# iiscleap/ICL-speech-text-LLM

Hardware: AMD Instinct MI355X
Metric: ICL utterances/sec (whole node), SALMONN+Llama2-7B 5-shot VOXCELEB (higher is better)
Workload: dtype bf16

## Files before the change

### icl-speech-text-llm_amd/csrc/gemm256.hip

```cpp
#include "gemm_common.h"
#include <cstdlib>

using namespace iclg;

#ifndef ICL_EPI_NT
#define ICL_EPI_NT 3
#endif

namespace {

constexpr int T256_REGION = 128 * 128;
constexpr int T256_BUF = 4 * T256_REGION;
constexpr int T256_SMEM = 256 * (256 * 2 + 16);

__device__ __forceinline__ void st16(unsigned short* dst, u32x4 v) {
  if (ICL_EPI_NT & 4) __builtin_nontemporal_store(v, (u32x4*)dst);
  else *(u32x4*)dst = v;
}

__device__ __forceinline__ void rope_rows(const GemmParams& p, const RopeFuse& rf, const char* smem, int pitch, int m0,
                                          int n0, int tid) {
  const int sect = n0 >= rf.v_off ? 2 : (n0 >= rf.k_off ? 1 : 0);
  const int head0 = (n0 - (sect == 2 ? rf.v_off : sect == 1 ? rf.k_off : 0)) >> 7;
  unsigned short* C = (unsigned short*)p.C;
  constexpr int U = 4;
  if (sect == 2) {
    for (int base = tid; base < 256 * 32; base += U * 512) {
      int64_t crow[U];
      if (rf.vc) {
#pragma unroll
        for (int u = 0; u < U; ++u) {
          const int m = min(m0 + ((base + u * 512) >> 5), p.M - 1);
          crow[u] = (int64_t)rf.seq_ids[m] * rf.H * rf.max_len + rf.pos[m];
        }
      }
#pragma unroll
      for (int u = 0; u < U; ++u) {
        const int c = base + u * 512, row = c >> 5, cc = c & 31, m = m0 + row;
        if (m >= p.M) continue;
        const u32x4 v = *(const u32x4*)(smem + row * pitch + cc * 16);
        if (rf.kv_rows_to_c) st16(C + (int64_t)m * p.ldc + n0 + cc * 8, v);
        if (rf.vc) st16(rf.vc + (crow[u] + (int64_t)(head0 + (cc >> 4)) * rf.max_len) * 128 + (cc & 15) * 8, v);
      }
    }
    return;
  }
  const bool to_cache = sect == 1 && rf.kc;
  for (int base = tid; base < 256 * 16; base += U * 512) {
    int ps[U], sq[U];
    u32x4 lo[U], hi[U];
    f32x4 c0[U], c1[U], s0[U], s1[U];
#pragma unroll
    for (int u = 0; u < U; ++u) {
      const int m = min(m0 + ((base + u * 512) >> 4), p.M - 1);
      ps[u] = rf.pos[m];
      sq[u] = to_cache ? rf.seq_ids[m] : 0;
    }
#pragma unroll
    for (int u = 0; u < U; ++u) {
      const int it = base + u * 512, row = it >> 4, hh = (it >> 3) & 1, j = it & 7;
      const char* src = smem + row * pitch + hh * 256 + j * 16;
      lo[u] = *(const u32x4*)src;
      hi[u] = *(const u32x4*)(src + 128);
      const float* cp = rf.cosT + (int64_t)ps[u] * 64 + j * 8;
      const float* sp = rf.sinT + (int64_t)ps[u] * 64 + j * 8;
      c0[u] = *(const f32x4*)cp;
      c1[u] = *(const f32x4*)(cp + 4);
      s0[u] = *(const f32x4*)sp;
      s1[u] = *(const f32x4*)(sp + 4);
    }
#pragma unroll
    for (int u = 0; u < U; ++u) {
      const int it = base + u * 512, row = it >> 4, hh = (it >> 3) & 1, j = it & 7, m = m0 + row;
      if (m >= p.M) continue;
      u32x4 olo, ohi;
      rope_rot8(lo[u], hi[u], c0[u], c1[u], s0[u], s1[u], olo, ohi);
      if (sect == 0 || rf.kv_rows_to_c) {
        unsigned short* dst = C + (int64_t)m * p.ldc + n0 + hh * 128 + j * 8;
        st16(dst, olo);
        st16(dst + 64, ohi);
      }
      if (to_cache) {
        unsigned short* cd = rf.kc + (((int64_t)sq[u] * rf.H + head0 + hh) * rf.max_len + ps[u]) * 128 + j * 8;
        st16(cd, olo);
        st16(cd + 64, ohi);
      }
    }
  }
}

constexpr int T256_OUT_F32 = 16;
template <bool ROPE, int EPI>
__global__ __launch_bounds__(512, 2) void gemm256_bf16_kernel(GemmParams p_in, RopeFuse rf) {
  GemmParams p = p_in;
  p.epi = (p_in.epi & ICL_EPI_BIAS) | (EPI & (ICL_EPI_GELU | ICL_EPI_RESIDUAL | ICL_EPI_SWIGLU));
  p.out_dtype = (EPI & T256_OUT_F32) ? ICL_F32 : ICL_BF16;
  extern __shared__ __attribute__((aligned(16))) char smem[];
  const int tid = threadIdx.x, lane = tid & 63;
  const int wave = __builtin_amdgcn_readfirstlane(tid >> 6);
  const int wr = wave >> 2, wc = wave & 3;
  int tm, tn;
  block_to_tile(p, blockIdx.x, tm, tn);
  const int m0 = tm * 256, n0 = tn * 256;
  int z = blockIdx.z;
  int nk = p.K >> 6, kt0 = 0;
  const bool slab_out = p.split_k > 1;
  if (p.split_k > 1) {
    kt0 = (int)(((int64_t)z * nk) / p.split_k);
    nk = (int)(((int64_t)(z + 1) * nk) / p.split_k) - kt0;
    p.C = p.ws + (int64_t)z * p.M * p.N;
    p.ldc = p.N;
    p.sC = 0;
    p.epi = 0;
    z = 0;
  }
  const __bf16* A = p.A + (int64_t)z * p.sA + (int64_t)kt0 * 64;
  const __bf16* Wk = p.W + (int64_t)kt0 * 64;

  const __bf16* gsrc[2][2][2];
#pragma unroll
  for (int h = 0; h < 2; ++h)
#pragma unroll
    for (int r = 0; r < 2; ++r) {
      const int row = (r * 8 + wave) * 8 + (lane >> 3);
      const int chunk = (lane & 7) ^ ((row >> 1) & 7);
      gsrc[0][h][r] = A + (int64_t)min(m0 + h * 128 + row, p.M - 1) * p.lda + chunk * 8;
      gsrc[1][h][r] = Wk + (int64_t)min(n0 + h * 128 + row, p.N - 1) * p.ldw + chunk * 8;
    }
  auto stage = [&](int bo, int which, int h, int kt) {
    const int64_t koff = (int64_t)min(kt, nk - 1) * 64;
    char* base = smem + bo + (which * 2 + h) * T256_REGION + wave * 1024;
    __builtin_amdgcn_global_load_lds((gptr_t)(gsrc[which][h][0] + koff), (lptr_t)(base), 16, 0, 0);
    __builtin_amdgcn_global_load_lds((gptr_t)(gsrc[which][h][1] + koff), (lptr_t)(base + 8 * 1024), 16, 0, 0);
  };

  const int fr = lane & 15, fq = lane >> 4;
  const int a_base = (wr * 64 + fr) * 128, b_base = (wc * 32 + fr) * 128;
  const int sw0 = ((0 + fq) ^ (fr >> 1)) * 16, sw1 = ((4 + fq) ^ (fr >> 1)) * 16;

  f32x4 acc[2][2][4][2];
#pragma unroll
  for (int a = 0; a < 2; ++a)
#pragma unroll
    for (int b = 0; b < 2; ++b)
#pragma unroll
      for (int i = 0; i < 4; ++i)
#pragma unroll
        for (int j = 0; j < 2; ++j) acc[a][b][i][j] = f32x4{0.f, 0.f, 0.f, 0.f};
  bf16x8 af[4][2], b0f[2][2], b1f[2][2];
  const bool vecp = vec_path_ok(p);
  const bool interior = vecp && (m0 + 256 <= p.M) && (n0 + 256 <= p.N);
  const bool fold_bias = vecp && (p.epi & ICL_EPI_BIAS);
  constexpr bool fold_res = false;

  auto read_a = [&](int bo, int h) {
    const char* r = smem + bo + h * T256_REGION + a_base;
#pragma unroll
    for (int i = 0; i < 4; ++i) {
      af[i][0] = *(const bf16x8*)(r + i * 2048 + sw0);
      af[i][1] = *(const bf16x8*)(r + i * 2048 + sw1);
    }
  };
  auto read_b = [&](int bo, int h, bf16x8 (&bf)[2][2]) {
    const char* r = smem + bo + (2 + h) * T256_REGION + b_base;
#pragma unroll
    for (int j = 0; j < 2; ++j) {
      bf[j][0] = *(const bf16x8*)(r + j * 2048 + sw0);
      bf[j][1] = *(const bf16x8*)(r + j * 2048 + sw1);
    }
  };
  auto mma = [&](f32x4 (&c)[4][2], bf16x8 (&bf)[2][2]) {
    __builtin_amdgcn_s_setprio(1);
#pragma unroll
    for (int kk = 0; kk < 2; ++kk)
#pragma unroll
      for (int i = 0; i < 4; ++i)
#pragma unroll
        for (int j = 0; j < 2; ++j)
          c[i][j] = __builtin_amdgcn_mfma_f32_16x16x32_bf16(bf[j][kk], af[i][kk], c[i][j], 0, 0, 0);
    __builtin_amdgcn_s_setprio(0);
    __builtin_amdgcn_sched_barrier(0);
    __builtin_amdgcn_s_barrier();
    __builtin_amdgcn_sched_barrier(0);
  };
  auto phase_sync = [&](auto n_tag) {
    constexpr int N = decltype(n_tag)::value;
    if constexpr (N == 8) asm volatile("s_waitcnt vmcnt(8)" ::: "memory");
    else if constexpr (N == 6) asm volatile("s_waitcnt vmcnt(6)" ::: "memory");
    else if constexpr (N == 4) asm volatile("s_waitcnt vmcnt(4)" ::: "memory");
    else if constexpr (N == 2) asm volatile("s_waitcnt vmcnt(2)" ::: "memory");
    else asm volatile("s_waitcnt vmcnt(0)" ::: "memory");
    __builtin_amdgcn_sched_barrier(0);
    __builtin_amdgcn_s_barrier();
    __builtin_amdgcn_sched_barrier(0);
  };
  auto tile = [&](int bo, int t, auto mode) {
    constexpr int MODE = decltype(mode)::value;
    const int bx = bo ^ T256_BUF;
    read_a(bo, 0);
    read_b(bo, 0, b0f);
    if constexpr (MODE != 2) stage(bx, 1, 1, t + 1);
    phase_sync(std::integral_constant<int, MODE == 2 ? 2 : 8>{});
    mma(acc[0][0], b0f);
    read_b(bo, 1, b1f);
    if constexpr (MODE != 2) stage(bx, 0, 1, t + 1);
    phase_sync(std::integral_constant<int, MODE == 2 ? 0 : 8>{});
    mma(acc[0][1], b1f);
    read_a(bo, 1);
    if constexpr (MODE == 0) stage(bo, 0, 0, t + 2);
    phase_sync(std::integral_constant<int, MODE == 0 ? 8 : (MODE == 1 ? 6 : 0)>{});
    mma(acc[1][1], b1f);
    if constexpr (MODE == 0) stage(bo, 1, 0, t + 2);
    phase_sync(std::integral_constant<int, MODE == 0 ? 8 : (MODE == 1 ? 4 : 0)>{});
    mma(acc[1][0], b0f);
  };
  using M0_ = std::integral_constant<int, 0>;
  using M1_ = std::integral_constant<int, 1>;
  using M2_ = std::integral_constant<int, 2>;

  f32x4 bias_f[2][2];
  if (fold_res) {
#pragma unroll
    for (int qa = 0; qa < 2; ++qa)
#pragma unroll
      for (int qb = 0; qb < 2; ++qb)
#pragma unroll
        for (int i = 0; i < 4; ++i)
#pragma unroll
          for (int j = 0; j < 2; ++j) {
            const int m = m0 + qa * 128 + wr * 64 + i * 16 + fr, n = n0 + qb * 128 + wc * 32 + j * 16 + fq * 4;
            if (interior || (m < p.M && n < p.N))
              acc[qa][qb][i][j] = *(const f32x4*)((const float*)p.R + (int64_t)z * p.sR + (int64_t)m * p.ldr + n);
          }
  }
  if (fold_bias) {
#pragma unroll
    for (int qb = 0; qb < 2; ++qb)
#pragma unroll
      for (int j = 0; j < 2; ++j) {
        const int n = n0 + qb * 128 + wc * 32 + j * 16 + fq * 4;
        bias_f[qb][j] = (interior || n < p.N) ? *(const f32x4*)(p.bias + n) : f32x4{0.f, 0.f, 0.f, 0.f};
      }
  }
  __builtin_amdgcn_sched_barrier(0);
  stage(0, 0, 0, 0);
  stage(0, 1, 0, 0);
  stage(0, 1, 1, 0);
  stage(0, 0, 1, 0);
  stage(T256_BUF, 0, 0, 1);
  stage(T256_BUF, 1, 0, 1);
  __builtin_amdgcn_sched_barrier(0);
  if (fold_bias) {
#pragma unroll
    for (int qa = 0; qa < 2; ++qa)
#pragma unroll
      for (int qb = 0; qb < 2; ++qb)
#pragma unroll
        for (int i = 0; i < 4; ++i)
#pragma unroll
          for (int j = 0; j < 2; ++j) acc[qa][qb][i][j] = acc[qa][qb][i][j] + bias_f[qb][j];
  }
  phase_sync(std::integral_constant<int, 8>{});
  if (wr == 1) __builtin_amdgcn_s_barrier();
  const int n_steady = nk - 2;
  int t = 0;
  for (; t + 1 < n_steady; t += 2) {
    tile(0, t, M0_{});
    tile(T256_BUF, t + 1, M0_{});
  }
  if (t < n_steady) {
    tile(0, t, M0_{});
    ++t;
  }
  const int bo = (t & 1) ? T256_BUF : 0;
  tile(bo, t, M1_{});
  tile(bo ^ T256_BUF, t + 1, M2_{});
  if (wr == 0) __builtin_amdgcn_s_barrier();

  const int es_out = p.out_dtype == ICL_BF16 ? 2 : 4;
  const bool rows16 = (((uintptr_t)p.C | (uintptr_t)(p.ldc * es_out) | (uintptr_t)(p.sC * es_out)) & 15) == 0;
  const bool has_res = p.epi & ICL_EPI_RESIDUAL;
  const bool res_rows = has_res && p.res_dtype == ICL_F32 && p.out_dtype == ICL_F32 && !(p.epi & ICL_EPI_SWIGLU) &&
                        (((uintptr_t)p.R | (uintptr_t)(p.ldr * 4) | (uintptr_t)(p.sR * 4)) & 15) == 0;
  if (ROPE || (interior && rows16 && (!has_res || res_rows))) {
    const bool swiglu = p.epi & ICL_EPI_SWIGLU;
    const bool obf = p.out_dtype == ICL_BF16;
    const int out_cols = swiglu ? 128 : 256;
    const int es = obf ? 2 : 4;
    const int pitch = out_cols * es + 16;
    const int chunks_per_row = out_cols * es / 16;
    const int64_t c_col0 = swiglu ? (n0 >> 1) : n0;
    const bool one_round = ROPE || obf;
    f32x4 rrA[16], rrB[16];
    auto load_res_rows = [&](int qa_, f32x4 (&rr)[16]) {
      const char* rbase = (const char*)p.R + ((int64_t)z * p.sR + (int64_t)(m0 + qa_ * 128) * p.ldr + n0) * 4;
#pragma unroll
      for (int it = 0; it < 16; ++it) {
        const int c = tid + it * 512, row = c >> 6, cc = c & 63;
        rr[it] = ICL_EPI_NT & 1 ? __builtin_nontemporal_load((const f32x4*)(rbase + (int64_t)row * p.ldr * 4 + cc * 16))
                                : *(const f32x4*)(rbase + (int64_t)row * p.ldr * 4 + cc * 16);
      }
    };
    if (has_res) load_res_rows(0, rrA);
#pragma unroll
    for (int qa = 0; qa < 2; ++qa) {
      if (qa == 0 || !one_round) __syncthreads();
      const int row_off = one_round ? qa * 128 : 0;
#pragma unroll
      for (int qb = 0; qb < 2; ++qb)
#pragma unroll
        for (int i = 0; i < 4; ++i) {
          const int row = row_off + wr * 64 + i * 16 + fr;
          if (swiglu) {
            f32x4 v;
#pragma unroll
            for (int r = 0; r < 4; ++r) v[r] = silu_f(acc[qa][qb][i][0][r]) * acc[qa][qb][i][1][r];
            const int col = qb * 64 + wc * 16 + fq * 4;
            char* dst = smem + row * pitch + col * es;
            if (obf) *(u32x2*)dst = u32x2{pack_bf16x2(v[0], v[1]), pack_bf16x2(v[2], v[3])};
            else *(f32x4*)dst = v;
          } else {
#pragma unroll
            for (int j = 0; j < 2; ++j) {
              f32x4 v = acc[qa][qb][i][j];
              if (p.epi & ICL_EPI_GELU) {
            v = gelu_erf4(v);
              }
              const int col = qb * 128 + wc * 32 + j * 16 + fq * 4;
              char* dst = smem + row * pitch + col * es;
              if (obf) *(u32x2*)dst = u32x2{pack_bf16x2(v[0], v[1]), pack_bf16x2(v[2], v[3])};
              else *(f32x4*)dst = v;
            }
          }
        }
      if (one_round && qa == 0) continue;
      __syncthreads();
      if constexpr (ROPE) {
        rope_rows(p, rf, smem, pitch, m0, n0, tid);
        continue;
      }
      char* cbase = (char*)p.C + ((int64_t)z * p.sC + (int64_t)(m0 + (one_round ? 0 : qa * 128)) * p.ldc + c_col0) * es;
      const int n_chunks = (one_round ? 256 : 128) * chunks_per_row;
      if (has_res) {
        if (qa == 0) load_res_rows(1, rrB);
        f32x4 (&rr)[16] = qa == 0 ? rrA : rrB;
#pragma unroll
        for (int it = 0; it < 16; ++it) {
          const int c = tid + it * 512, row = c >> 6, cc = c & 63;
          const f32x4 v = *(const f32x4*)(smem + row * pitch + cc * 16) + rr[it];
          if (ICL_EPI_NT & 1) __builtin_nontemporal_store(v, (f32x4*)(cbase + (int64_t)row * p.ldc * 4 + cc * 16));
          else *(f32x4*)(cbase + (int64_t)row * p.ldc * 4 + cc * 16) = v;
        }
      } else {
        const int n_iter = n_chunks >> 9;
        u32x4 v[16];
#pragma unroll
        for (int it = 0; it < 16; ++it)
          if (it < n_iter) {
            const int c = tid + it * 512, row = c / chunks_per_row, cc = c - row * chunks_per_row;
            v[it] = *(const u32x4*)(smem + row * pitch + cc * 16);
          }
#pragma unroll
        for (int it = 0; it < 16; ++it)
          if (it < n_iter) {
            const int c = tid + it * 512, row = c / chunks_per_row, cc = c - row * chunks_per_row;
            if ((ICL_EPI_NT & 2) && !slab_out) __builtin_nontemporal_store(v[it], (u32x4*)(cbase + (int64_t)row * p.ldc * es + cc * 16));
            else *(u32x4*)(cbase + (int64_t)row * p.ldc * es + cc * 16) = v[it];
          }
      }
    }
    return;
  } else if (interior) {
    const bool late_res = (p.epi & ICL_EPI_RESIDUAL) && !fold_res;
#pragma unroll
    for (int qa = 0; qa < 2; ++qa) {
      const int mb = m0 + qa * 128 + wr * 64 + fr;
      if (p.epi & ICL_EPI_SWIGLU) {
#pragma unroll
        for (int i = 0; i < 4; ++i)
#pragma unroll
          for (int qb = 0; qb < 2; ++qb) {
            f32x4 v;
#pragma unroll
            for (int r = 0; r < 4; ++r) v[r] = silu_f(acc[qa][qb][i][0][r]) * acc[qa][qb][i][1][r];
            store_out4(p, (int64_t)z * p.sC + (int64_t)(mb + i * 16) * p.ldc + ((n0 + qb * 128 + wc * 32) >> 1) + fq * 4, v);
          }
        continue;
      }
      f32x4 rv[2][4][2];
      if (late_res) {
#pragma unroll
        for (int qb = 0; qb < 2; ++qb)
#pragma unroll
          for (int i = 0; i < 4; ++i)
#pragma unroll
            for (int j = 0; j < 2; ++j)
              rv[qb][i][j] = load_res4(p, (int64_t)z * p.sR + (int64_t)(mb + i * 16) * p.ldr + n0 + qb * 128 + wc * 32 + j * 16 + fq * 4);
      }
#pragma unroll
      for (int qb = 0; qb < 2; ++qb)
#pragma unroll
        for (int i = 0; i < 4; ++i)
#pragma unroll
          for (int j = 0; j < 2; ++j) {
            f32x4 v = acc[qa][qb][i][j];
            if (p.epi & ICL_EPI_GELU) {
            v = gelu_erf4(v);
            }
            if (late_res) v = v + rv[qb][i][j];
            store_out4(p, (int64_t)z * p.sC + (int64_t)(mb + i * 16) * p.ldc + n0 + qb * 128 + wc * 32 + j * 16 + fq * 4, v);
          }
    }
    return;
  }

  GemmParams q = p;
  if (fold_bias) q.epi &= ~ICL_EPI_BIAS;
  if (fold_res) q.epi &= ~ICL_EPI_RESIDUAL;
#pragma unroll
  for (int qa = 0; qa < 2; ++qa)
#pragma unroll
    for (int i = 0; i < 4; ++i) {
      const int m = m0 + qa * 128 + wr * 64 + i * 16 + fr;
#pragma unroll
      for (int qb = 0; qb < 2; ++qb) {
        const int nt = n0 + qb * 128 + wc * 32;
        if (p.epi & ICL_EPI_SWIGLU) {
          epi_store_swiglu(q, z, m, nt, fq * 4, acc[qa][qb][i][0], acc[qa][qb][i][1]);
        } else {
          epi_store4(q, z, m, nt + fq * 4, acc[qa][qb][i][0]);
          epi_store4(q, z, m, nt + 16 + fq * 4, acc[qa][qb][i][1]);
        }
      }
    }
}

template <bool ROPE, int EPI>
int launch256(const GemmParams& p, const dim3& grid, hipStream_t stream, const RopeFuse& rf) {
  auto kern = gemm256_bf16_kernel<ROPE, EPI>;
  static bool attr_set = false;
  if (!attr_set) {
    const hipError_t e = hipFuncSetAttribute((const void*)kern, hipFuncAttributeMaxDynamicSharedMemorySize, T256_SMEM);
    if (e != hipSuccess) {
      icl_set_error("icl_gemm_bf16: hipFuncSetAttribute(%d) failed: %s", T256_SMEM, hipGetErrorString(e));
      return ICL_ELAUNCH;
    }
    attr_set = true;
  }
  hipLaunchKernelGGL(kern, grid, dim3(512), T256_SMEM, stream, p, rf);
  ICL_CHECK_LAUNCH("icl_gemm_bf16(256)");
  return ICL_OK;
}

}

int iclg::launch_tile256(GemmParams& p, int batch, hipStream_t stream, const RopeFuse* rope) {
  p.tiles_m = (p.M + 255) / 256;
  p.tiles_n = (p.N + 255) / 256;
  {
    static const int env_gm = [] { const char* e = getenv("ICL_GEMM_GROUP_M"); return e ? atoi(e) : 0; }();
    static const int env_xs = [] { const char* e = getenv("ICL_GEMM_XCD_SYNC"); return e ? atoi(e) : 1; }();
    const int64_t panel = (int64_t)256 * p.K * 2;
    p.group_m = env_gm > 0 ? env_gm : (int)std::min<int64_t>(6, std::max<int64_t>(1, 8400000 / panel));
    p.xcd_sync = env_xs;
  }
  const dim3 grid(p.tiles_m * p.tiles_n, 1, p.split_k > 1 ? p.split_k : batch);
  if (rope) return launch256<true, 0>(p, grid, stream, *rope);
  const RopeFuse none{};
  constexpr int G = ICL_EPI_GELU, R = ICL_EPI_RESIDUAL, S = ICL_EPI_SWIGLU, F = T256_OUT_F32;
  if (p.split_k > 1) return launch256<false, F>(p, grid, stream, none);
  switch ((p.epi & (G | R | S)) | (p.out_dtype == ICL_F32 ? F : 0)) {
    case 0:         return launch256<false, 0>(p, grid, stream, none);
    case G:         return launch256<false, G>(p, grid, stream, none);
    case R:         return launch256<false, R>(p, grid, stream, none);
    case G | R:     return launch256<false, G | R>(p, grid, stream, none);
    case S:         return launch256<false, S>(p, grid, stream, none);
    case F:         return launch256<false, F>(p, grid, stream, none);
    case F | G:     return launch256<false, F | G>(p, grid, stream, none);
    case F | R:     return launch256<false, F | R>(p, grid, stream, none);
    case F | G | R: return launch256<false, F | G | R>(p, grid, stream, none);
    case F | S:     return launch256<false, F | S>(p, grid, stream, none);
  }
  icl_set_error("icl_gemm_bf16(256): unsupported epilogue combination 0x%x", p.epi);
  return ICL_EINVAL;
}
```

Measured before the change: 143.2.

## Make 256-tile GEMM persistent and overlap next tile prologue with epilogue stores

Turns the 256x256 GEMM kernel into a persistent kernel: the grid is capped at the CU count and each workgroup loops over tiles with stride gridDim.x. During the row-store epilogue of one tile, it resets the accumulators, loads the bias and issues the first global-to-LDS loads for the next tile. A new pipeline mode accounts for the extra outstanding stores in vmcnt. This hides the prologue latency and launch tail, but adds complexity and a fixed CU-count grid, which can unbalance the last wave of tiles.

```diff
diff --git a/icl-speech-text-llm_amd/csrc/gemm256.hip b/icl-speech-text-llm_amd/csrc/gemm256.hip
--- a/icl-speech-text-llm_amd/csrc/gemm256.hip
+++ b/icl-speech-text-llm_amd/csrc/gemm256.hip
@@ -95,13 +95,12 @@
   GemmParams p = p_in;
   p.epi = (p_in.epi & ICL_EPI_BIAS) | (EPI & (ICL_EPI_GELU | ICL_EPI_RESIDUAL | ICL_EPI_SWIGLU));
   p.out_dtype = (EPI & T256_OUT_F32) ? ICL_F32 : ICL_BF16;
+  constexpr int S_AFTER = ROPE ? 0 : ((EPI & T256_OUT_F32 ? 128 : 256) * ((EPI & ICL_EPI_SWIGLU ? 128 : 256) * (EPI & T256_OUT_F32 ? 4 : 2) / 16)) >> 9;
   extern __shared__ __attribute__((aligned(16))) char smem[];
-  const int tid = threadIdx.x, lane = tid & 63;
-  const int wave = __builtin_amdgcn_readfirstlane(tid >> 6);
+  const int wave = __builtin_amdgcn_readfirstlane(threadIdx.x >> 6);
   const int wr = wave >> 2, wc = wave & 3;
-  int tm, tn;
-  block_to_tile(p, blockIdx.x, tm, tn);
-  const int m0 = tm * 256, n0 = tn * 256;
+  const int nwg = p.tiles_m * p.tiles_n;
+  int bid = blockIdx.x;
   int z = blockIdx.z;
   int nk = p.K >> 6, kt0 = 0;
   const bool slab_out = p.split_k > 1;
@@ -117,16 +116,42 @@
   const __bf16* A = p.A + (int64_t)z * p.sA + (int64_t)kt0 * 64;
   const __bf16* Wk = p.W + (int64_t)kt0 * 64;
 
+  const bool vecp = vec_path_ok(p);
+  const bool fold_bias = vecp && (p.epi & ICL_EPI_BIAS);
+  constexpr bool fold_res = false;
+
+  int m0, n0;
+  bool interior;
   const __bf16* gsrc[2][2][2];
-#pragma unroll
-  for (int h = 0; h < 2; ++h)
-#pragma unroll
-    for (int r = 0; r < 2; ++r) {
-      const int row = (r * 8 + wave) * 8 + (lane >> 3);
-      const int chunk = (lane & 7) ^ ((row >> 1) & 7);
-      gsrc[0][h][r] = A + (int64_t)min(m0 + h * 128 + row, p.M - 1) * p.lda + chunk * 8;
-      gsrc[1][h][r] = Wk + (int64_t)min(n0 + h * 128 + row, p.N - 1) * p.ldw + chunk * 8;
-    }
+  f32x4 bias_f[2][2];
+  auto tile_begin = [&](int b) {
+    int tid = threadIdx.x;
+    asm volatile("" : "+v"(tid));
+    const int lane = tid & 63, fq = lane >> 4;
+    int tm, tn;
+    block_to_tile(p, b, tm, tn);
+    m0 = __builtin_amdgcn_readfirstlane(tm * 256);
+    n0 = __builtin_amdgcn_readfirstlane(tn * 256);
+    interior = vecp && (m0 + 256 <= p.M) && (n0 + 256 <= p.N);
+#pragma unroll
+    for (int h = 0; h < 2; ++h)
+#pragma unroll
+      for (int r = 0; r < 2; ++r) {
+        const int row = (r * 8 + wave) * 8 + (lane >> 3);
+        const int chunk = (lane & 7) ^ ((row >> 1) & 7);
+        gsrc[0][h][r] = A + (int64_t)min(m0 + h * 128 + row, p.M - 1) * p.lda + chunk * 8;
+        gsrc[1][h][r] = Wk + (int64_t)min(n0 + h * 128 + row, p.N - 1) * p.ldw + chunk * 8;
+      }
+    if (fold_bias) {
+#pragma unroll
+      for (int qb = 0; qb < 2; ++qb)
+#pragma unroll
+        for (int j = 0; j < 2; ++j) {
+          const int n = n0 + qb * 128 + wc * 32 + j * 16 + fq * 4;
+          bias_f[qb][j] = (interior || n < p.N) ? *(const f32x4*)(p.bias + n) : f32x4{0.f, 0.f, 0.f, 0.f};
+        }
+    }
+  };
   auto stage = [&](int bo, int which, int h, int kt) {
     const int64_t koff = (int64_t)min(kt, nk - 1) * 64;
     char* base = smem + bo + (which * 2 + h) * T256_REGION + wave * 1024;
@@ -134,24 +159,26 @@
     __builtin_amdgcn_global_load_lds((gptr_t)(gsrc[which][h][1] + koff), (lptr_t)(base + 8 * 1024), 16, 0, 0);
   };
 
+  const int lane = threadIdx.x & 63;
   const int fr = lane & 15, fq = lane >> 4;
   const int a_base = (wr * 64 + fr) * 128, b_base = (wc * 32 + fr) * 128;
   const int sw0 = ((0 + fq) ^ (fr >> 1)) * 16, sw1 = ((4 + fq) ^ (fr >> 1)) * 16;
 
   f32x4 acc[2][2][4][2];
-#pragma unroll
-  for (int a = 0; a < 2; ++a)
-#pragma unroll
-    for (int b = 0; b < 2; ++b)
-#pragma unroll
-      for (int i = 0; i < 4; ++i)
-#pragma unroll
-        for (int j = 0; j < 2; ++j) acc[a][b][i][j] = f32x4{0.f, 0.f, 0.f, 0.f};
   bf16x8 af[4][2], b0f[2][2], b1f[2][2];
-  const bool vecp = vec_path_ok(p);
-  const bool interior = vecp && (m0 + 256 <= p.M) && (n0 + 256 <= p.N);
-  const bool fold_bias = vecp && (p.epi & ICL_EPI_BIAS);
-  constexpr bool fold_res = false;
+  auto acc_init = [&] {
+#pragma unroll
+    for (int qa = 0; qa < 2; ++qa)
+#pragma unroll
+      for (int qb = 0; qb < 2; ++qb)
+#pragma unroll
+        for (int i = 0; i < 4; ++i)
+#pragma unroll
+          for (int j = 0; j < 2; ++j) {
+            acc[qa][qb][i][j] = f32x4{0.f, 0.f, 0.f, 0.f};
+            if (fold_bias) acc[qa][qb][i][j] = acc[qa][qb][i][j] + bias_f[qb][j];
+          }
+  };
 
   auto read_a = [&](int bo, int h) {
     const char* r = smem + bo + h * T256_REGION + a_base;
@@ -185,11 +212,8 @@
   };
   auto phase_sync = [&](auto n_tag) {
     constexpr int N = decltype(n_tag)::value;
-    if constexpr (N == 8) asm volatile("s_waitcnt vmcnt(8)" ::: "memory");
-    else if constexpr (N == 6) asm volatile("s_waitcnt vmcnt(6)" ::: "memory");
-    else if constexpr (N == 4) asm volatile("s_waitcnt vmcnt(4)" ::: "memory");
-    else if constexpr (N == 2) asm volatile("s_waitcnt vmcnt(2)" ::: "memory");
-    else asm volatile("s_waitcnt vmcnt(0)" ::: "memory");
+    static_assert(N >= 0 && N <= 63, "vmcnt is a 6-bit field on gfx950");
+    asm volatile("s_waitcnt vmcnt(%0)" ::"n"(N) : "memory");
     __builtin_amdgcn_sched_barrier(0);
     __builtin_amdgcn_s_barrier();
     __builtin_amdgcn_sched_barrier(0);
@@ -199,89 +223,46 @@
     const int bx = bo ^ T256_BUF;
     read_a(bo, 0);
     read_b(bo, 0, b0f);
+    constexpr int W8 = MODE == 3 ? 8 + S_AFTER : 8;
     if constexpr (MODE != 2) stage(bx, 1, 1, t + 1);
-    phase_sync(std::integral_constant<int, MODE == 2 ? 2 : 8>{});
+    phase_sync(std::integral_constant<int, MODE == 2 ? 2 : W8>{});
     mma(acc[0][0], b0f);
     read_b(bo, 1, b1f);
     if constexpr (MODE != 2) stage(bx, 0, 1, t + 1);
-    phase_sync(std::integral_constant<int, MODE == 2 ? 0 : 8>{});
+    phase_sync(std::integral_constant<int, MODE == 2 ? 0 : W8>{});
     mma(acc[0][1], b1f);
     read_a(bo, 1);
-    if constexpr (MODE == 0) stage(bo, 0, 0, t + 2);
-    phase_sync(std::integral_constant<int, MODE == 0 ? 8 : (MODE == 1 ? 6 : 0)>{});
+    if constexpr (MODE == 0 || MODE == 3) stage(bo, 0, 0, t + 2);
+    phase_sync(std::integral_constant<int, MODE == 0 || MODE == 3 ? W8 : (MODE == 1 ? 6 : 0)>{});
     mma(acc[1][1], b1f);
-    if constexpr (MODE == 0) stage(bo, 1, 0, t + 2);
-    phase_sync(std::integral_constant<int, MODE == 0 ? 8 : (MODE == 1 ? 4 : 0)>{});
+    if constexpr (MODE == 0 || MODE == 3) stage(bo, 1, 0, t + 2);
+    phase_sync(std::integral_constant<int, MODE == 0 || MODE == 3 ? W8 : (MODE == 1 ? 4 : 0)>{});
     mma(acc[1][0], b0f);
   };
   using M0_ = std::integral_constant<int, 0>;
   using M1_ = std::integral_constant<int, 1>;
   using M2_ = std::integral_constant<int, 2>;
-
-  f32x4 bias_f[2][2];
-  if (fold_res) {
-#pragma unroll
-    for (int qa = 0; qa < 2; ++qa)
-#pragma unroll
-      for (int qb = 0; qb < 2; ++qb)
-#pragma unroll
-        for (int i = 0; i < 4; ++i)
-#pragma unroll
-          for (int j = 0; j < 2; ++j) {
-            const int m = m0 + qa * 128 + wr * 64 + i * 16 + fr, n = n0 + qb * 128 + wc * 32 + j * 16 + fq * 4;
-            if (interior || (m < p.M && n < p.N))
-              acc[qa][qb][i][j] = *(const f32x4*)((const float*)p.R + (int64_t)z * p.sR + (int64_t)m * p.ldr + n);
-          }
-  }
-  if (fold_bias) {
-#pragma unroll
-    for (int qb = 0; qb < 2; ++qb)
-#pragma unroll
-      for (int j = 0; j < 2; ++j) {
-        const int n = n0 + qb * 128 + wc * 32 + j * 16 + fq * 4;
-        bias_f[qb][j] = (interior || n < p.N) ? *(const f32x4*)(p.bias + n) : f32x4{0.f, 0.f, 0.f, 0.f};
-      }
-  }
-  __builtin_amdgcn_sched_barrier(0);
-  stage(0, 0, 0, 0);
-  stage(0, 1, 0, 0);
-  stage(0, 1, 1, 0);
-  stage(0, 0, 1, 0);
-  stage(T256_BUF, 0, 0, 1);
-  stage(T256_BUF, 1, 0, 1);
-  __builtin_amdgcn_sched_barrier(0);
-  if (fold_bias) {
-#pragma unroll
-    for (int qa = 0; qa < 2; ++qa)
-#pragma unroll
-      for (int qb = 0; qb < 2; ++qb)
-#pragma unroll
-        for (int i = 0; i < 4; ++i)
-#pragma unroll
-          for (int j = 0; j < 2; ++j) acc[qa][qb][i][j] = acc[qa][qb][i][j] + bias_f[qb][j];
-  }
-  phase_sync(std::integral_constant<int, 8>{});
-  if (wr == 1) __builtin_amdgcn_s_barrier();
-  const int n_steady = nk - 2;
-  int t = 0;
-  for (; t + 1 < n_steady; t += 2) {
-    tile(0, t, M0_{});
-    tile(T256_BUF, t + 1, M0_{});
-  }
-  if (t < n_steady) {
-    tile(0, t, M0_{});
-    ++t;
-  }
-  const int bo = (t & 1) ? T256_BUF : 0;
-  tile(bo, t, M1_{});
-  tile(bo ^ T256_BUF, t + 1, M2_{});
-  if (wr == 0) __builtin_amdgcn_s_barrier();
+  using M3_ = std::integral_constant<int, 3>;
+
+  auto prologue = [&] {
+    __builtin_amdgcn_sched_barrier(0);
+    stage(0, 0, 0, 0);
+    stage(0, 1, 0, 0);
+    stage(0, 1, 1, 0);
+    stage(0, 0, 1, 0);
+    stage(T256_BUF, 0, 0, 1);
+    stage(T256_BUF, 1, 0, 1);
+    __builtin_amdgcn_sched_barrier(0);
+  };
 
   const int es_out = p.out_dtype == ICL_BF16 ? 2 : 4;
   const bool rows16 = (((uintptr_t)p.C | (uintptr_t)(p.ldc * es_out) | (uintptr_t)(p.sC * es_out)) & 15) == 0;
   const bool has_res = p.epi & ICL_EPI_RESIDUAL;
   const bool res_rows = has_res && p.res_dtype == ICL_F32 && p.out_dtype == ICL_F32 && !(p.epi & ICL_EPI_SWIGLU) &&
                         (((uintptr_t)p.R | (uintptr_t)(p.ldr * 4) | (uintptr_t)(p.sR * 4)) & 15) == 0;
+  auto epilogue = [&](const bool more, const int nbid) -> bool {
+  int tid = threadIdx.x;
+  asm volatile("" : "+v"(tid));
   if (ROPE || (interior && rows16 && (!has_res || res_rows))) {
     const bool swiglu = p.epi & ICL_EPI_SWIGLU;
     const bool obf = p.out_dtype == ICL_BF16;
@@ -302,6 +283,14 @@
       }
     };
     if (has_res) load_res_rows(0, rrA);
+    const bool prefetch = !ROPE && more && nk >= 4;
+    auto next_prologue = [&] {
+      acc_init();
+      asm volatile("s_waitcnt lgkmcnt(0)" ::: "memory");
+      __builtin_amdgcn_sched_barrier(0);
+      __builtin_amdgcn_s_barrier();
+      prologue();
+    };
 #pragma unroll
     for (int qa = 0; qa < 2; ++qa) {
       if (qa == 0 || !one_round) __syncthreads();
@@ -334,22 +323,30 @@
           }
         }
       if (one_round && qa == 0) continue;
+      char* cbase = (char*)p.C + ((int64_t)z * p.sC + (int64_t)(m0 + (one_round ? 0 : qa * 128)) * p.ldc + c_col0) * es;
+      const bool last = one_round || qa == 1;
+      if (last && prefetch) tile_begin(nbid);
       __syncthreads();
       if constexpr (ROPE) {
         rope_rows(p, rf, smem, pitch, m0, n0, tid);
         continue;
       }
-      char* cbase = (char*)p.C + ((int64_t)z * p.sC + (int64_t)(m0 + (one_round ? 0 : qa * 128)) * p.ldc + c_col0) * es;
       const int n_chunks = (one_round ? 256 : 128) * chunks_per_row;
       if (has_res) {
         if (qa == 0) load_res_rows(1, rrB);
         f32x4 (&rr)[16] = qa == 0 ? rrA : rrB;
+        f32x4 v[16];
 #pragma unroll
         for (int it = 0; it < 16; ++it) {
           const int c = tid + it * 512, row = c >> 6, cc = c & 63;
-          const f32x4 v = *(const f32x4*)(smem + row * pitch + cc * 16) + rr[it];
-          if (ICL_EPI_NT & 1) __builtin_nontemporal_store(v, (f32x4*)(cbase + (int64_t)row * p.ldc * 4 + cc * 16));
-          else *(f32x4*)(cbase + (int64_t)row * p.ldc * 4 + cc * 16) = v;
+          v[it] = *(const f32x4*)(smem + row * pitch + cc * 16) + rr[it];
+        }
+        if (last && prefetch) next_prologue();
+#pragma unroll
+        for (int it = 0; it < 16; ++it) {
+          const int c = tid + it * 512, row = c >> 6, cc = c & 63;
+          if (ICL_EPI_NT & 1) __builtin_nontemporal_store(v[it], (f32x4*)(cbase + (int64_t)row * p.ldc * 4 + cc * 16));
+          else *(f32x4*)(cbase + (int64_t)row * p.ldc * 4 + cc * 16) = v[it];
         }
       } else {
         const int n_iter = n_chunks >> 9;
@@ -360,6 +357,9 @@
             const int c = tid + it * 512, row = c / chunks_per_row, cc = c - row * chunks_per_row;
             v[it] = *(const u32x4*)(smem + row * pitch + cc * 16);
           }
+        static_assert(ROPE || S_AFTER == ((EPI & T256_OUT_F32 ? 128 : 256) * ((EPI & ICL_EPI_SWIGLU ? 128 : 256) * (EPI & T256_OUT_F32 ? 4 : 2) / 16) >> 9),
+                      "S_AFTER = the row stores a thread issues in the last row phase (n_iter below)");
+        if (last && prefetch) next_prologue();
 #pragma unroll
         for (int it = 0; it < 16; ++it)
           if (it < n_iter) {
@@ -369,7 +369,7 @@
           }
       }
     }
-    return;
+    return prefetch;
   } else if (interior) {
     const bool late_res = (p.epi & ICL_EPI_RESIDUAL) && !fold_res;
 #pragma unroll
@@ -411,7 +411,7 @@
             store_out4(p, (int64_t)z * p.sC + (int64_t)(mb + i * 16) * p.ldc + n0 + qb * 128 + wc * 32 + j * 16 + fq * 4, v);
           }
     }
-    return;
+    return false;
   }
 
   GemmParams q = p;
@@ -433,6 +433,47 @@
         }
       }
     }
+  return false;
+  };
+
+  bool pre = false;
+  for (;;) {
+    const int nbid = __builtin_amdgcn_readfirstlane(bid + (int)gridDim.x);
+    const bool more = nbid < nwg;
+    if (!(!ROPE && pre)) {
+      tile_begin(bid);
+      prologue();
+      acc_init();
+      phase_sync(std::integral_constant<int, 8>{});
+    } else {
+      phase_sync(std::integral_constant<int, 8 + S_AFTER>{});
+    }
+    if (wr == 1) __builtin_amdgcn_s_barrier();
+    const int n_steady = nk - 2;
+    int t = 0;
+    if (!ROPE && pre) {
+      tile(0, 0, M3_{});
+      tile(T256_BUF, 1, M0_{});
+      t = 2;
+    }
+    for (; t + 1 < n_steady; t += 2) {
+      tile(0, t, M0_{});
+      tile(T256_BUF, t + 1, M0_{});
+    }
+    if (t < n_steady) {
+      tile(0, t, M0_{});
+      ++t;
+    }
+    const int bo = (t & 1) ? T256_BUF : 0;
+    tile(bo, t, M1_{});
+    tile(bo ^ T256_BUF, t + 1, M2_{});
+    if (wr == 0) __builtin_amdgcn_s_barrier();
+
+    pre = __builtin_amdgcn_readfirstlane((int)epilogue(more, nbid)) != 0;
+    if (!more) break;
+    if (!pre) __syncthreads();
+    bid = nbid;
+  }
 }
 
 template <bool ROPE, int EPI>
@@ -452,6 +493,11 @@
   return ICL_OK;
 }
 
+bool persist_default(const GemmParams& p, bool rope) {
+  (void)p;
+  return !rope;
+}
+
 }
 
 int iclg::launch_tile256(GemmParams& p, int batch, hipStream_t stream, const RopeFuse* rope) {
@@ -464,7 +510,16 @@
     p.group_m = env_gm > 0 ? env_gm : (int)std::min<int64_t>(6, std::max<int64_t>(1, 8400000 / panel));
     p.xcd_sync = env_xs;
   }
-  const dim3 grid(p.tiles_m * p.tiles_n, 1, p.split_k > 1 ? p.split_k : batch);
+  static const int env_ps = [] { const char* e = getenv("ICL_GEMM_PERSIST"); return e ? atoi(e) : -1; }();
+  static const int n_cu = [] {
+    int dev = 0, n = 0;
+    if (hipGetDevice(&dev) != hipSuccess || hipDeviceGetAttribute(&n, hipDeviceAttributeMultiprocessorCount, dev) != hipSuccess) return 0;
+    return n;
+  }();
+  int gx = p.tiles_m * p.tiles_n;
+  const bool persist_ok = p.split_k <= 1 && p.K >= 256 && n_cu > 0 && (n_cu & 7) == 0 && gx > n_cu;
+  if (persist_ok && (env_ps > 0 || (env_ps < 0 && persist_default(p, rope != nullptr)))) gx = n_cu;
+  const dim3 grid(gx, 1, p.split_k > 1 ? p.split_k : batch);
   if (rope) return launch256<true, 0>(p, grid, stream, *rope);
   const RopeFuse none{};
   constexpr int G = ICL_EPI_GELU, R = ICL_EPI_RESIDUAL, S = ICL_EPI_SWIGLU, F = T256_OUT_F32;
```

Result: slower. 99.56, median of 2 (-30.5%).
